# microsoft/VidTok

Hardware: NVIDIA H100
Metric: frames/sec encode+decode, kl_causal_488 17x256x256 (higher is better)
Workload: dtype bf16

## Files before the change

### vidtok_b200/csrc/conv_tc.cu

```cuda
#include <cuda.h>

#include <cstdio>
#include <cstdlib>
#include <cstring>
#include <mutex>
#include <string>
#include <type_traits>

#include "common.cuh"
#include "kernels.h"
#include "tc_host.h"
#include "tc_ptx.cuh"

namespace vt {

namespace {

thread_local std::string g_tc_err;

struct TcParams {
  int B, To, Ho, Wo, Co, Ti;
  int BW, BH, BT;
  int tilesW, tilesH, tilesT;
  int num_n_tiles, BN;
// ... 7 lines not shown
  int res_mode;
  const bf16* res;
  long long rsB, rsT, rsH, rsW;
  int resT, res_t_mode, res_pool_off;
  const bf16* res_cache;
  float ra, rb;
  void* out;
  long long osB, osT, osH, osW, osC;
  int out_f32;
  int Co_real;
  int w_batched;
  int ln_mode, ln_silu;
  const float* ln_gamma;
  const float* ln_beta;
  void* out2;
  int res_mma;
  int halo, hP, a_stages;
  uint32_t halo_bytes;
  int split, a_lo, b_lo, o_lo;
  float acc_scale;
  int kparts;
  int reg_mode, reg_zc, reg_sample;
  const float* reg_noise;
  float* reg_z;
  int* reg_idx;
  double* reg_kl;
  FsqConst reg_fsq;
  uint32_t misc_off;
  int stage_out;
  uint32_t stage_smem;
  uint32_t stage_off;
  int half_dim, half_ext;
  int relu;
};

struct TcMaps {
  CUtensorMap a[4];
  CUtensorMap c;
  CUtensorMap b;
  CUtensorMap r;
  CUtensorMap e;
  CUtensorMap o, o2;
};

constexpr int kConsumerWarps = 8;
constexpr int kProducerWarp = kConsumerWarps;
constexpr int kThreads = (kConsumerWarps + 4) * 32;
constexpr int kABytes = 128 * 128;
constexpr uint32_t kBarTurn = 3, kBarBias = 5, kBarStage = 7;
constexpr uint32_t kStageOutBytes = 64 * 128;

__host__ __device__ constexpr bool ping_pong(int BN, bool split) { return !split && (BN == 64 || BN == 128); }

using namespace tcx;

struct TileCoord {
  int b, t0, h0, w0, n0;
};
__device__ __forceinline__ TileCoord decode_tile(const TcParams& p, long long tile) {
  TileCoord c;
  const int nt = (int)(tile % p.num_n_tiles);
  long long m = tile / p.num_n_tiles;
  const int tw = (int)(m % p.tilesW); m /= p.tilesW;
  const int th = (int)(m % p.tilesH); m /= p.tilesH;
  const int tt = (int)(m % p.tilesT);
  c.b = (int)(m / p.tilesT);
  c.t0 = tt * p.BT; c.h0 = th * p.BH; c.w0 = tw * p.BW; c.n0 = nt * p.BN;
  return c;
}
__device__ __forceinline__ bool tap_time(const TcParams& p, const TileCoord& tc, int a, int& tv, bool& from_cache) {
  tv = (tc.t0 + p.to_off) * p.st + a - p.pt;
  from_cache = false;
  if (tv + p.BT <= 0) {
    if (p.t_mode == 0) return false;
    if (p.t_mode == 1) { tv = 0; return true; }
    from_cache = true;
    tv = p.cacheT + tv;
    return true;
  }
  return true;
}
__device__ __forceinline__ int tile_taps(const TcParams& p, const TileCoord& tc) {
  int n = 0;
  for (int a = 0; a < p.kt; ++a) {
    int tv;
    bool from_cache;
    if (tap_time(p, tc, a, tv, from_cache)) ++n;
  }
  return n;
}

__device__ __forceinline__ float quad_sum(float v) {
  v += __shfl_xor_sync(0xffffffffu, v, 1);
  v += __shfl_xor_sync(0xffffffffu, v, 2);
  return v;
}

template <int BN, bool kSplit, bool kStage = false>
__global__ void __launch_bounds__(kThreads, 1)
conv_tc_kernel(const __grid_constant__ TcMaps maps, const TcParams p) {
  extern __shared__ uint8_t smem_raw[];
  const uint32_t smem_base = (smem_u32(smem_raw) + 1023u) & ~1023u;
  uint8_t* smem_gen = smem_raw + (smem_base - smem_u32(smem_raw));
  const int warp = threadIdx.x >> 5, lane = threadIdx.x & 31;
  const uint32_t a_bytes = kABytes;
  constexpr uint32_t b_bytes = (uint32_t)BN * 128u;
  constexpr uint32_t kPl = kSplit ? 2u : 1u;
  const uint32_t stage_bytes = kPl * (p.halo ? b_bytes : a_bytes + b_bytes);
  const uint32_t win_bytes = kPl * p.halo_bytes;
  const uint32_t ring_base = smem_base + (p.halo ? (uint32_t)p.a_stages * win_bytes : 0u);
  const uint32_t bar_base = ring_base + p.stages * stage_bytes + p.stage_smem;
  auto full_bar = [&](int s) { return bar_base + 8u * s; };
  auto empty_bar = [&](int s) { return bar_base + 8u * (p.stages + s); };
// ... 171 lines not shown
    pend_stage = stage;
    pend_win = last_of_window;
    if (++stage == nstages) { stage = 0; phase ^= 1u; }
  };

  const int rbase = (kPingPong ? 0 : 64 * g) + 16 * wq + (lane >> 2);
  const int cq = 2 * (lane & 3);
  const bool res_direct = (p.res_mode == 1 && !p.res_mma);
  const bool store_a = (p.ln_mode != 1);
  const float inv_n = 1.0f / (float)BN;
  int last_n0 = -1;
  uint32_t cbuf = 1;

  int owner = 0;
  for (long long tile = blockIdx.x; tile < p.num_tiles; tile += gridDim.x, owner ^= 1) {
    const TileCoord tc = decode_tile(p, tile);
    if constexpr (kPingPong) {
      if (owner != g) {
        const int taps = tile_taps(p, tc);
        stage += taps * nsp * num_kc + res_steps;
        if ((stage / nstages) & 1) phase ^= 1u;
        stage %= nstages;
        if (halo) {
          const int nw = taps * num_kc + res_steps;
          sA += nw;
          if ((sA / p.a_stages) & 1) phA ^= 1u;
          sA %= p.a_stages;
          sR = (sR + nw) % p.a_stages;
        }
        continue;
      }
      if (tile != blockIdx.x) named_bar_sync(kBarTurn + g, kConsumerWarps * 32);
    }
    uint32_t G = 0xFFFFFFFFu;
    if constexpr (kSum) {
      if (p.kparts > 1) {
        const uint32_t nk = (uint32_t)(tile_taps(p, tc) * nsp * num_kc + res_steps);
        G = (nk + (uint32_t)p.kparts - 1u) / (uint32_t)p.kparts;
      }
#pragma unroll
      for (int i = 0; i < R; ++i) sum[i] = 0.f;
    }
    uint32_t ks = 0, accum = 0;
    auto step = [&](bool a_from_stage, uint32_t a_addr, bool res, bool last_of_window) {
      if constexpr (kSum) {
        if (ks > 0 && ks % G == 0) {
          wgmma_wait<0>();
          acc_fence(acc[0]);
          release();
#pragma unroll
          for (int i = 0; i < R; ++i) sum[i] += acc[0][i];
          accum = 0;
        }
      }
      kstep(a_from_stage, a_addr, accum, res, last_of_window);
      accum = 1;
      ++ks;
    };
    for (int a = 0; a < p.kt; ++a) {
      int tv;
      bool from_cache;
      if (!tap_time(p, tc, a, tv, from_cache)) continue;
      if (halo) {
        for (int kc = 0; kc < num_kc; ++kc) {
          mbar_wait(fullA_bar(sA), phA);
          const uint32_t win = smem_base + (uint32_t)sA * win_bytes + a_row_off;
// ... 19 lines not shown
      if (tile + gridDim.x < p.num_tiles) named_bar_arrive(kBarTurn + (g ^ 1), kConsumerWarps * 32);
    }
    wgmma_wait<0>();
#pragma unroll
    for (int hf = 0; hf < kHalves; ++hf) acc_fence(acc[hf]);
    release();
    if constexpr (kSum) {
#pragma unroll
      for (int i = 0; i < R; ++i) acc[0][i] += sum[i];
    }

    if (tc.n0 != last_n0) {
      last_n0 = tc.n0;
      cbuf ^= 1u;
      constexpr int nthr = kPingPong ? 128 : kConsumerWarps * 32;
      float* b_ = sbias + ((kPingPong ? 2 * g : 0) + cbuf) * 768;
      for (int i = threadIdx.x % nthr; i < BN; i += nthr) {
        b_[i] = (p.bias && tc.n0 + i < p.Co_real) ? p.bias[tc.n0 + i] : 0.f;
        if (p.ln_mode) { const float sc = (p.ln_silu && !kSplit) ? 0.5f : 1.0f; b_[256 + i] = sc * p.ln_gamma[tc.n0 + i]; b_[512 + i] = sc * p.ln_beta[tc.n0 + i]; }
      }
      named_bar_sync(kPingPong ? kBarBias + g : 1u, nthr);
    }
    const float* bias_s = sbias + ((kPingPong ? 2 * g : 0) + cbuf) * 768;
    const float* gamma_s = bias_s + 256;
    const float* beta_s = bias_s + 512;

#pragma unroll
    for (int hf = 0; hf < kHalves; ++hf) {
      float (&acc_h)[R] = acc[hf];
      int row0 = rbase + 64 * hf;
      asm volatile("" : "+r"(row0));
      bool valid[2];
      long long ooff[2];
      auto row_geom = [&](int row, int& t, int& h, int& w) {
        const int dw = halo ? (row & 7) : row % p.BW;
        const int dh = halo ? (row >> 3) : (row / p.BW) % p.BH;
        const int dt = halo ? 0 : row / (p.BW * p.BH);
        t = tc.t0 + dt; h = tc.h0 + dh; w = tc.w0 + dw;
        return (t < p.To) && (h < p.Ho) && (w < p.Wo);
      };
#pragma unroll
      for (int r = 0; r < 2; ++r) {
        int t, h, w;
        valid[r] = row_geom(row0 + 8 * r, t, h, w);
        ooff[r] = (long long)tc.b * p.osB + (long long)t * p.osT + (long long)h * p.osH + (long long)w * p.osW;
      }
      auto res_pair = [&](const bf16* rp, int c, float& x0, float& x1) {
        const uint32_t hw = *reinterpret_cast<const uint32_t*>(rp + c);
        if constexpr (kSplit) {
          const uint32_t lw = *reinterpret_cast<const uint32_t*>(rp + p.o_lo + c);
          x0 = f16_lo(hw) + f16_lo(lw);
          x1 = f16_hi(hw) + f16_hi(lw);
        } else {
          x0 = bf16_lo(hw);
          x1 = bf16_hi(hw);
        }
      };
#pragma unroll
      for (int j = 0; j < BN / 8; ++j) {
        const int c = 8 * j + cq;
#pragma unroll
        for (int e = 0; e < 4; ++e) {
          float f = kSplit ? fmaf(acc_h[4 * j + e], p.acc_scale, bias_s[c + (e & 1)]) : acc_h[4 * j + e] + bias_s[c + (e & 1)];
          if (p.rb != 1.0f) f *= p.rb;
          acc_h[4 * j + e] = f;
        }
      }
      if (res_direct || p.res_mode == 3) {
#pragma unroll
        for (int r = 0; r < 2; ++r) {
          int t, h, w;
          if (!row_geom(row0 + 8 * r, t, h, w)) continue;
          const bf16* r0 = nullptr;
          const bf16* r1 = nullptr;
          const bf16* r2 = nullptr;
          if (res_direct) {
            r0 = p.res + (long long)tc.b * p.rsB + (long long)t * p.rsT + (long long)h * p.rsH + (long long)w * p.rsW + tc.n0;
          } else {
            const long long sp = (long long)tc.b * p.rsB + (long long)h * p.rsH + (long long)w * p.rsW + tc.n0;
            const int ta = 2 * t - 1 + p.res_pool_off, tb = ta + 1, tcn = ta + 2;
            if (ta >= 0) r0 = p.res + sp + (long long)ta * p.rsT;
            else if (p.res_t_mode == 1) r0 = p.res + sp;
            else if (p.res_t_mode == 2) r0 = p.res_cache + (((long long)tc.b * p.Ho + h) * p.Wo + w) * (long long)p.Co * (kSplit ? 2 : 1) + tc.n0;
            if (tb < p.resT) r1 = p.res + sp + (long long)tb * p.rsT;
            if (tcn < p.resT) r2 = p.res + sp + (long long)tcn * p.rsT;
          }
#pragma unroll
          for (int j = 0; j < BN / 8; ++j) {
            const int c = 8 * j + cq;
            if (res_direct) {
              float x0, x1;
              res_pair(r0, c, x0, x1);
              acc_h[4 * j + 2 * r] = fmaf(p.ra, x0, acc_h[4 * j + 2 * r]);
              acc_h[4 * j + 2 * r + 1] = fmaf(p.ra, x1, acc_h[4 * j + 2 * r + 1]);
            } else {
              float s0 = 0.f, s1 = 0.f, x0, x1;
              if (r0) { res_pair(r0, c, x0, x1); s0 += x0; s1 += x1; }
              if (r1) { res_pair(r1, c, x0, x1); s0 += x0; s1 += x1; }
              if (r2) { res_pair(r2, c, x0, x1); s0 += x0; s1 += x1; }
              const float s3 = p.ra * (1.0f / 3.0f);
              acc_h[4 * j + 2 * r] = fmaf(s3, s0, acc_h[4 * j + 2 * r]);
              acc_h[4 * j + 2 * r + 1] = fmaf(s3, s1, acc_h[4 * j + 2 * r + 1]);
            }
          }
        }
// ... 119 lines not shown
              reserve();
#pragma unroll
              for (int r = 0; r < 2; ++r)
#pragma unroll
                for (int u = 0; u < 8; ++u) put_s(r, u, pack_bf16x2(acc_h[4 * (8 * k + u) + 2 * r], acc_h[4 * (8 * k + u) + 2 * r + 1]));
              send(&maps.o, k);
            }
          }
          if (p.ln_mode) {
            const CUtensorMap* nmap = p.ln_mode == 1 ? &maps.o : &maps.o2;
#pragma unroll
            for (int k = 0; k < BN / 64; ++k) {
              reserve();
#pragma unroll
              for (int r = 0; r < 2; ++r)
#pragma unroll
                for (int u = 0; u < 8; ++u) {
                  const int j = 8 * k + u, c = 8 * j + cq;
                  float y0 = fmaf(fmaf(acc_h[4 * j + 2 * r], rstd[r], nmr[r]), gamma_s[c], beta_s[c]);
                  float y1 = fmaf(fmaf(acc_h[4 * j + 2 * r + 1], rstd[r], nmr[r]), gamma_s[c + 1], beta_s[c + 1]);
                  if (p.ln_silu) {
                    y0 = fmaf(y0, tanh_approx(y0), y0);
                    y1 = fmaf(y1, tanh_approx(y1), y1);
                  }
                  put_s(r, u, pack_bf16x2(y0, y1));
                }
              send(nmap, k);
            }
          }
          continue;
        }
      }

      auto put = [&](void* optr, int r, int c, float y0, float y1) {
        bf16* o = reinterpret_cast<bf16*>(optr) + ooff[r] + tc.n0 + c;
        if constexpr (kSplit) {
          const uint32_t hw = pack_f16x2(y0, y1);
          *reinterpret_cast<uint32_t*>(o) = hw;
          *reinterpret_cast<uint32_t*>(o + p.o_lo) = pack_f16x2(y0 - f16_lo(hw), y1 - f16_hi(hw));
        } else {
          *reinterpret_cast<uint32_t*>(o) = pack_bf16x2(y0, y1);
        }
      };
      if constexpr (kSplit) {
        if (store_a) {
#pragma unroll
          for (int r = 0; r < 2; ++r)
            if (valid[r])
#pragma unroll
              for (int j = 0; j < BN / 8; ++j) put(p.out, r, 8 * j + cq, acc_h[4 * j + 2 * r], acc_h[4 * j + 2 * r + 1]);
        }
        if (p.ln_mode) {
          void* nout = p.ln_mode == 1 ? p.out : p.out2;
#pragma unroll
          for (int r = 0; r < 2; ++r) {
            float s = 0.f;
#pragma unroll
            for (int j = 0; j < BN / 8; ++j) s += acc_h[4 * j + 2 * r] + acc_h[4 * j + 2 * r + 1];
            const float mean = quad_sum(s) * inv_n;
            float q = 0.f;
#pragma unroll
            for (int j = 0; j < BN / 8; ++j) {
              const float d0 = acc_h[4 * j + 2 * r] - mean, d1 = acc_h[4 * j + 2 * r + 1] - mean;
              q = fmaf(d0, d0, q);
              q = fmaf(d1, d1, q);
            }
            const float rstd = 1.0f / sqrtf(quad_sum(q) * inv_n + 1e-6f);
            if (!valid[r]) continue;
#pragma unroll
            for (int j = 0; j < BN / 8; ++j) {
              const int c = 8 * j + cq;
              float y0 = (acc_h[4 * j + 2 * r] - mean) * rstd * gamma_s[c] + beta_s[c];
              float y1 = (acc_h[4 * j + 2 * r + 1] - mean) * rstd * gamma_s[c + 1] + beta_s[c + 1];
              if (p.ln_silu) { y0 = silu_tc(y0); y1 = silu_tc(y1); }
              put(nout, r, c, y0, y1);
            }
          }
        }
      } else {
#pragma unroll
        for (int r = 0; r < 2; ++r) {
          float s = 0.f, q = 0.f;
#pragma unroll
          for (int j = 0; j < BN / 8; ++j) {
            const float f0 = acc_h[4 * j + 2 * r], f1 = acc_h[4 * j + 2 * r + 1];
            s += f0 + f1;
            q = fmaf(f0, f0, q);
            q = fmaf(f1, f1, q);
            const uint32_t kp = pack_bf16x2(f0, f1);
            if (store_a && valid[r]) *reinterpret_cast<uint32_t*>(reinterpret_cast<bf16*>(p.out) + ooff[r] + tc.n0 + 8 * j + cq) = kp;
            acc_h[4 * j + 2 * r] = bf16_lo(kp);
            acc_h[4 * j + 2 * r + 1] = bf16_hi(kp);
          }
          if (!p.ln_mode) continue;
          const float mean = quad_sum(s) * inv_n;
          float var = fmaf(-mean, mean, quad_sum(q) * inv_n);
          var = var < 0.f ? 0.f : var;
          const float rstd = rsqrtf(var + 1e-6f);
          const float nmr = -mean * rstd;
          if (!valid[r]) continue;
          void* nout = p.ln_mode == 1 ? p.out : p.out2;
#pragma unroll
          for (int j = 0; j < BN / 8; ++j) {
            const int c = 8 * j + cq;
            float y0 = fmaf(fmaf(acc_h[4 * j + 2 * r], rstd, nmr), gamma_s[c], beta_s[c]);
            float y1 = fmaf(fmaf(acc_h[4 * j + 2 * r + 1], rstd, nmr), gamma_s[c + 1], beta_s[c + 1]);
            if (p.ln_silu) {
              y0 = fmaf(y0, tanh_approx(y0), y0);
              y1 = fmaf(y1, tanh_approx(y1), y1);
            }
            put(nout, r, c, y0, y1);
          }
        }
      }
    }
  }
  if (kStage && (threadIdx.x & 127) == 0) bulk_wait<0>();
}

__global__ void fill_identity_kernel(bf16* e, int f16, float value) {
  const int r = blockIdx.x, c = threadIdx.x;
  if (f16) reinterpret_cast<__half*>(e)[r * 256 + c] = __float2half_rn(r == c ? value : 0.0f);
  else e[r * 256 + c] = __float2bfloat16_rn(r == c ? value : 0.0f);
}

bool choose_tile(const ConvP& p, int rows, int& BW, int& BH, int& BT) {
  const bool allow_bt = (p.st == 1) && (p.t_mode == 0);
  long long best = -1;
  auto ceil_to = [](int v, int b) { return (long long)((v + b - 1) / b) * b; };
  for (int bw = 128; bw >= 8; bw >>= 1) {
    for (int bh = rows / bw; bh >= 1; bh >>= 1) {
      if (bh > 256) continue;
      const int bt = rows / (bw * bh);
      if (bt > 1 && !allow_bt) continue;
      if (bt > 16) continue;
      const long long padded = ceil_to(p.Wo, bw) * ceil_to(p.Ho, bh) * ceil_to(p.To, bt);
      const long long cost = padded * 1024 + (long long)(bw > 16 ? bw - 16 : 16 - bw) * 4 + (bt - 1);
      if (best < 0 || cost < best) { best = cost; BW = bw; BH = bh; BT = bt; }
    }
  }
  return best >= 0;
}
int choose_bn(int Co) {
  for (int bn = 256; bn >= 32; bn >>= 1)
// ... 84 lines not shown
  if (rc == 1) rc = plan(false, bn_pref);
  if (rc == 1 && !need_row) rc = plan(false, 128);
  if (rc == 1) return no("not enough shared memory for 2 stages");
  if (rc != 0) return false;
  bool ident_ok = true;
  if (split) {
    const float ws = p.acc_scale != 0.f ? 1.0f / p.acc_scale : 1.0f;
    t.ident_s = ilogbf(ws);
    ident_ok = t.ident_s >= 0 && t.ident_s <= 15 && ldexpf(1.0f, t.ident_s) == ws;
  }
  t.res_mma = (ident_ok && p.res_mode == 1 && p.ra == 1.0f && p.rb == 1.0f && t.BN % 64 == 0 && p.Co % 64 == 0 && p.rsW % 8 == 0 &&
               p.rsH % 8 == 0 && p.rsT % 8 == 0 && p.rsB % 8 == 0 && (((uintptr_t)p.res) & 15) == 0) ? 1 : 0;
  *out = t;
  return true;
}

cudaError_t launch_conv_tc(const TcPlan& pl, const bf16* x, const bf16* w_nk, void* out, cudaStream_t s, long long w_batch_stride) {
  if (!tmap_encoder()) { g_tc_err = "cuTensorMapEncodeTiled unavailable"; return cudaErrorNotSupported; }
  const ConvP& p = pl.p;
  const TcRegFusion& reg = pl.reg;
  const bool split = p.split != 0;
  const int cw = split ? 2 : 1;
  if (reg.mode ? (!reg.z || (reg.mode == 1 && (!reg.kl_acc || (reg.sample && !reg.noise)))) : !out) { g_tc_err = "null output"; return cudaErrorInvalidValue; }
  if (p.t_mode == 2 && (!p.cache || p.cacheT <= 0)) { g_tc_err = "cache mode without cache"; return cudaErrorInvalidValue; }
  int dev = 0;
  const cudaError_t dev_err = current_device(dev);
  if (dev_err != cudaSuccess) { g_tc_err = "no current device, or its index is out of range"; return dev_err; }
  const int Co_pad = (p.Co + 31) / 32 * 32, Kpad = p.kt * p.kh * p.kw * p.Ci;
  TcParams t;
  memset(&t, 0, sizeof(t));
  t.BW = pl.BW; t.BH = pl.BH; t.BT = pl.BT; t.BN = pl.BN;
  t.halo = pl.halo; t.hP = pl.hP; t.a_stages = pl.a_stages; t.halo_bytes = pl.halo_bytes;
  t.stages = pl.stages; t.misc_off = pl.misc_off; t.kparts = pl.kparts; t.res_mma = pl.res_mma;
  t.stage_smem = pl.stage_out ? 2 * kStageOutBytes : 0;
  t.stage_off = (uint32_t)pl.a_stages * pl.halo_bytes + (uint32_t)pl.stages * (uint32_t)((pl.halo ? 0 : kABytes) + pl.BN * 128);
  t.stage_out = (pl.stage_out && ((uintptr_t)out & 15) == 0 && ((uintptr_t)pl.ln.out2 & 15) == 0) ? 1 : 0;
  t.tilesW = (p.Wo + t.BW - 1) / t.BW; t.tilesH = (p.Ho + t.BH - 1) / t.BH; t.tilesT = (p.To + t.BT - 1) / t.BT;
  t.num_n_tiles = Co_pad / t.BN;
  t.num_tiles = (long long)p.B * t.tilesT * t.tilesH * t.tilesW * t.num_n_tiles;
  t.split = split ? 1 : 0; t.a_lo = p.Ci; t.b_lo = Kpad; t.o_lo = pl.o_lo ? pl.o_lo : p.Co;
  t.acc_scale = (split && p.acc_scale != 0.f) ? p.acc_scale : 1.0f;
  t.B = p.B; t.To = p.To; t.Ho = p.Ho; t.Wo = p.Wo; t.Co = p.Co; t.Ti = p.Ti;
  t.kt = p.kt; t.kh = p.kh; t.kw = p.kw; t.Ci = p.Ci; t.num_kc = p.Ci / 64;
  t.st = p.st; t.pt = p.pt; t.ph = p.ph; t.pw = p.pw; t.to_off = p.to_off; t.sp = p.sh;
  t.t_mode = p.t_mode; t.cacheT = p.cacheT;
  t.bias = p.bias; t.res_mode = p.res_mode; t.res = (const bf16*)p.res;
  t.rsB = p.rsB; t.rsT = p.rsT; t.rsH = p.rsH; t.rsW = p.rsW; t.resT = p.resT; t.res_t_mode = p.res_t_mode; t.res_pool_off = p.res_pool_off;
  t.res_cache = (const bf16*)p.res_cache; t.ra = p.ra; t.rb = p.rb;
  t.out = out; t.osB = p.osB; t.osT = p.osT; t.osH = p.osH; t.osW = p.osW; t.osC = p.osC;
  t.out_f32 = (pl.tout == DT_F32) ? 1 : 0;
  t.Co_real = p.Co;
  t.ln_mode = pl.ln.mode; t.ln_silu = pl.ln.silu ? 1 : 0; t.ln_gamma = pl.ln.gamma; t.ln_beta = pl.ln.beta; t.out2 = pl.ln.out2;
  if (reg.mode) {
    t.reg_mode = reg.mode; t.reg_zc = reg.zc; t.reg_sample = reg.sample; t.reg_noise = reg.noise; t.reg_z = reg.z;
    t.reg_idx = reg.indices; t.reg_kl = reg.kl_acc;
    if (reg.mode == 2) t.reg_fsq = make_fsq_const(reg.zc, reg.fsq_levels);
  }
  t.w_batched = pl.w_batches > 1 ? 1 : 0;
  t.relu = p.relu ? 1 : 0;

  TcMaps maps;
  auto encode_act = [&](CUtensorMap* m, const bf16* base, int Wn, int Hn, long long sw_, long long sh_, int Tn, long long st_, long long bs) -> bool {
    cuuint64_t dims[5] = {(cuuint64_t)(cw * p.Ci), (cuuint64_t)Wn, (cuuint64_t)Hn, (cuuint64_t)Tn, (cuuint64_t)p.B};
    cuuint64_t strides[4] = {(cuuint64_t)sw_ * 2, (cuuint64_t)sh_ * 2, (cuuint64_t)st_ * 2, (cuuint64_t)bs * 2};
    cuuint32_t box[5] = {64, (cuuint32_t)t.BW, (cuuint32_t)t.BH, (cuuint32_t)t.BT, 1};
    if (t.halo) { box[1] = (cuuint32_t)t.hP; box[2] = (cuuint32_t)(16 + p.kh - 1); }
    return encode_tmap_16b(m, 5, base, dims, strides, box, "activation", g_tc_err);
  };
  if (p.sh == 1) {
    if (!encode_act(&maps.a[0], x, p.Wi, p.Hi, p.isW, p.isH, p.Ti, p.isT, p.isB)) return cudaErrorInvalidValue;
    maps.a[1] = maps.a[2] = maps.a[3] = maps.a[0];
  } else {
    for (int hp = 0; hp < 2; ++hp)
      for (int wp = 0; wp < 2; ++wp)
        if (!encode_act(&maps.a[hp * 2 + wp], x + (long long)hp * p.isH + (long long)wp * p.isW, (p.Wi - wp + 1) / 2,
                        (p.Hi - hp + 1) / 2, 2 * p.isW, 2 * p.isH, p.Ti, p.isT, p.isB))
          return cudaErrorInvalidValue;
  }
  if (p.t_mode == 2) {
    if (!encode_act(&maps.c, (const bf16*)p.cache, p.Wi, p.Hi, p.isW, p.isH, p.cacheT, p.isT, (long long)p.cacheT * p.Hi * p.Wi * p.Ci * cw)) return cudaErrorInvalidValue;
  } else {
// ... 81 lines not shown
```

### vidtok_b200/csrc/tblock_tc.cu

```cuda
#include <cuda.h>

#include <cstdio>
#include <cstring>
#include <string>

#include "common.cuh"
#include "kernels.h"
#include "tc_host.h"
#include "tc_ptx.cuh"

namespace vt {

namespace {
using namespace tcx;

thread_local std::string g_tb_err;
constexpr int kC = 128;
constexpr int kKc = kC / 64;
constexpr uint32_t kTile = 128 * 128;
constexpr int kHSlots = 3;
constexpr int kConsumerWarps = 8;
constexpr int kProducerWarp = kConsumerWarps;
constexpr int kThreadsTb = (kConsumerWarps + 4) * 32;

struct TbParams {
  int B, T, H, W;
  int BW, BH;
  int tilesW, tilesH;
  long long num_strips;
  int stages;
  const float* bias1;
  const float* bias2;
  const float* g2;
  const float* b2;
  int ln_out, ln_out_silu;
  const float* g3;
  const float* b3;
  const bf16* x;
  bf16* out;
  bf16* out2;
  const bf16* n1;
  int cached_in;
  const bf16* cn1_in;
  const bf16* ch_in;
  bf16* cn1_out;
  bf16* ch_out;
};
struct TbMaps {
  CUtensorMap n1, w1, w2, cn1;
  CUtensorMap x, out;
};

__device__ __forceinline__ float quad_sum(float v) {
  v += __shfl_xor_sync(0xffffffffu, v, 1);
  v += __shfl_xor_sync(0xffffffffu, v, 2);
  return v;
}

template <bool kCache>
__global__ void __launch_bounds__(kThreadsTb, 1) tblock_tc_kernel(const __grid_constant__ TbMaps maps, const TbParams p) {
  extern __shared__ uint8_t smem_raw[];
  const uint32_t smem_base = (smem_u32(smem_raw) + 1023u) & ~1023u;
  uint8_t* smem_gen = smem_raw + (smem_base - smem_u32(smem_raw));
  const int warp = threadIdx.x >> 5, lane = threadIdx.x & 31;
  const uint32_t h_base = smem_base;
  const uint32_t ring_base = h_base + kHSlots * kKc * kTile;
  const uint32_t stage_bytes = 2u * kTile;
  const uint32_t bar_base = ring_base + (uint32_t)p.stages * stage_bytes;
  auto full_bar = [&](int s) { return bar_base + 8u * s; };
  auto empty_bar = [&](int s) { return bar_base + 8u * (p.stages + s); };
  auto x_bar = [&](int g) { return bar_base + 16u * p.stages + 8u * g; };
  float* cst = reinterpret_cast<float*>(smem_gen + (bar_base - smem_base) + 16u * p.stages + 16u);

// ... 200 lines not shown
      finish();
      mbar_wait(x_bar(g), xphase);
      xphase ^= 1u;
      const uint32_t xslot = slot_of(t - 2);
#pragma unroll
      for (int r = 0; r < 2; ++r) {
        const long long off = (pos0[r] + (long long)t * frame) * kC;
        const int row = rbase + 8 * r;
        uint8_t* xs = smem_gen + (xslot - smem_base);
        float s = 0.f, q = 0.f;
#pragma unroll
        for (int j = 0; j < kC / 8; ++j) {
          const int c = 8 * j + cq;
          const int cc = c & 63;
          uint32_t* xo = reinterpret_cast<uint32_t*>(xs + (c >> 6) * kTile + swz128_unit(row, cc >> 3) + (cc & 7) * 2);
          const uint32_t xw = *xo;
          const float f0 = acc[4 * j + 2 * r] + bias2[c] + bf16_lo(xw), f1 = acc[4 * j + 2 * r + 1] + bias2[c + 1] + bf16_hi(xw);
          s += f0 + f1;
          q = fmaf(f0, f0, q);
          q = fmaf(f1, f1, q);
          const uint32_t kp = pack_bf16x2(f0, f1);
          *xo = kp;
          acc[4 * j + 2 * r] = bf16_lo(kp);
          acc[4 * j + 2 * r + 1] = bf16_hi(kp);
        }
        if (!p.ln_out) continue;
        const float mean = quad_sum(s) * (1.0f / kC);
        float var = fmaf(-mean, mean, quad_sum(q) * (1.0f / kC));
        var = var < 0.f ? 0.f : var;
        const float rstd = rsqrtf(var + 1e-6f);
        const float nmr = -mean * rstd;
        bf16* o2 = p.out2 + off;
#pragma unroll
        for (int j = 0; j < kC / 8; ++j) {
          const int c = 8 * j + cq;
          float y0 = fmaf(fmaf(acc[4 * j + 2 * r], rstd, nmr), g3[c], b3[c]);
          float y1 = fmaf(fmaf(acc[4 * j + 2 * r + 1], rstd, nmr), g3[c + 1], b3[c + 1]);
          if (p.ln_out_silu) {
            y0 = fmaf(y0, tanh_approx(y0), y0);
            y1 = fmaf(y1, tanh_approx(y1), y1);
          }
          *reinterpret_cast<uint32_t*>(o2 + c) = pack_bf16x2(y0, y1);
        }
      }
      fence_async_smem();
      wg_sync();
      if (gtid == 0) {
        for (int kc = 0; kc < kKc; ++kc)
          tma_store_5d(&maps.out, xslot + (uint32_t)g * 64u * 128u + (uint32_t)kc * kTile, kc * 64, box_w, box_h, t, b);
        bulk_commit();
      }
    }
    if (kCache) {
      for (int j = 0; j < 2; ++j) {
        const int tv = p.T - 2 + j;
        for (int i = gtid; i < 64 * 16; i += 128) {
          int row;
          const long long off = cache_pos(i, j, row);
          const long long pix = off - (((long long)b * 2 + j) * frame) * kC;
          uint4 hv = make_uint4(0u, 0u, 0u, 0u), nv = hv;
          if (tv >= 0 || front) hv = *ring_unit(slot_of(tv), row, (i & 15) * 8);
          if (tv >= 0) nv = *reinterpret_cast<const uint4*>(p.n1 + (((long long)b * p.T + tv) * frame) * kC + pix);
          else if (front) nv = *reinterpret_cast<const uint4*>(p.cn1_in + (((long long)b * 2 + tv + 2) * frame) * kC + pix);
          *reinterpret_cast<uint4*>(p.ch_out + off) = hv;
          *reinterpret_cast<uint4*>(p.cn1_out + off) = nv;
        }
      }
    }
  }
  if (gtid == 0) bulk_wait<0>();
}

bool strip_box(int H, int W, int& BW, int& BH) {
  for (int bw = 128; bw >= 1; bw >>= 1) {
    if (W % bw != 0) continue;
// ... 2 lines not shown
  }
  return false;
}
}

const char* tblock_tc_last_error() { return g_tb_err.c_str(); }

bool tblock_tc_supported(int B, int T, int H, int W, int C) {
  g_tb_err.clear();
  if (C != kC) { g_tb_err = "C != 128"; return false; }
  if (B <= 0 || T <= 0) { g_tb_err = "empty"; return false; }
  int BW, BH;
  if (!strip_box(H, W, BW, BH)) { g_tb_err = "H x W not tileable by a 128-position box"; return false; }
  return true;
}

cudaError_t launch_tblock_tc(const bf16* n1, const bf16* x, const bf16* w1, const float* bias1, const float* gamma2,
                             const float* beta2, const bf16* w2, const float* bias2, bf16* out, bf16* out2,
                             const float* gamma_out, const float* beta_out, bool out_silu, int B, int T, int H, int W,
                             cudaStream_t s, const TbCache* cache) {
  g_tb_err.clear();
  if (!tmap_encoder()) { g_tb_err = "cuTensorMapEncodeTiled unavailable"; return cudaErrorNotSupported; }
  TbParams p;
  memset(&p, 0, sizeof(p));
  if (!strip_box(H, W, p.BW, p.BH)) { g_tb_err = "H x W not tileable"; return cudaErrorInvalidValue; }
  p.B = B; p.T = T; p.H = H; p.W = W;
  p.tilesW = W / p.BW; p.tilesH = H / p.BH;
  p.num_strips = (long long)B * p.tilesH * p.tilesW;
  p.bias1 = bias1; p.bias2 = bias2; p.g2 = gamma2; p.b2 = beta2;
  p.ln_out = (out2 && gamma_out && beta_out) ? 1 : 0;
  p.ln_out_silu = out_silu ? 1 : 0;
  p.g3 = gamma_out; p.b3 = beta_out;
  p.x = x; p.out = out; p.out2 = out2;
  if (cache) {
    if (!cache->n1_out || !cache->h_out || (!cache->n1_in != !cache->h_in)) { g_tb_err = "cache: both outputs, and both or no inputs"; return cudaErrorInvalidValue; }
    p.n1 = n1;
    p.cached_in = cache->n1_in ? 1 : 0;
    p.cn1_in = cache->n1_in; p.ch_in = cache->h_in; p.cn1_out = cache->n1_out; p.ch_out = cache->h_out;
  }
  const size_t fixed = 1024 + (size_t)kHSlots * kKc * kTile + 16 + 6 * kC * 4;
  const size_t budget = 225 * 1024;
  int stages = (int)((budget - fixed) / (2 * kTile + 16));
  if (stages > 4) stages = 4;
  p.stages = stages;
  const size_t smem = fixed + (size_t)stages * (2 * kTile + 16);
  TbMaps maps;
  {
    cuuint64_t dims[5] = {(cuuint64_t)kC, (cuuint64_t)W, (cuuint64_t)H, (cuuint64_t)T, (cuuint64_t)B};
    cuuint64_t strides[4] = {(cuuint64_t)kC * 2, (cuuint64_t)W * kC * 2, (cuuint64_t)H * W * kC * 2, (cuuint64_t)T * H * W * kC * 2};
    cuuint32_t box[5] = {64, (cuuint32_t)p.BW, (cuuint32_t)p.BH, 1, 1};
    if (!encode_tmap_16b(&maps.n1, 5, n1, dims, strides, box, "n1", g_tb_err)) return cudaErrorInvalidValue;
    maps.cn1 = maps.n1;
    const int bw = p.BW < 64 ? p.BW : 64;
    cuuint32_t box64[5] = {64, (cuuint32_t)bw, (cuuint32_t)(64 / bw), 1, 1};
    for (int i = 0; i < 2; ++i)
      if (!encode_tmap_16b(i ? &maps.out : &maps.x, 5, i ? (const void*)out : x, dims, strides, box64, "x / out", g_tb_err))
        return cudaErrorInvalidValue;
    if (p.cached_in) {
      dims[3] = 2;
      strides[3] = 2ull * H * W * kC * 2;
      if (!encode_tmap_16b(&maps.cn1, 5, p.cn1_in, dims, strides, box, "n1 cache", g_tb_err)) return cudaErrorInvalidValue;
    }
  }
  for (int i = 0; i < 2; ++i) {
    cuuint64_t dims[3] = {(cuuint64_t)(3 * kC), (cuuint64_t)kC, 1};
    cuuint64_t strides[2] = {(cuuint64_t)(3 * kC) * 2, (cuuint64_t)(3 * kC) * kC * 2};
// ... 26 lines not shown
```

### vidtok_b200/csrc/tc_ptx.cuh

```cuda
#pragma once
#include <cuda.h>
#include <cuda_bf16.h>
#include <cuda_fp16.h>
#include <stdint.h>

namespace vt {
namespace tcx {
__device__ __forceinline__ uint32_t smem_u32(const void* p) { return (uint32_t)__cvta_generic_to_shared(p); }

__device__ __forceinline__ void mbar_init(uint32_t bar, uint32_t count) {
  asm volatile("mbarrier.init.shared::cta.b64 [%0], %1;" ::"r"(bar), "r"(count) : "memory");
}
__device__ __forceinline__ void mbar_expect_tx(uint32_t bar, uint32_t bytes) {
  asm volatile("mbarrier.arrive.expect_tx.shared::cta.b64 _, [%0], %1;" ::"r"(bar), "r"(bytes) : "memory");
}
__device__ __forceinline__ void mbar_arrive(uint32_t bar) {
  asm volatile("mbarrier.arrive.shared::cta.b64 _, [%0];" ::"r"(bar) : "memory");
}
__device__ __forceinline__ bool mbar_try_wait(uint32_t bar, uint32_t parity) {
  uint32_t ok;
  asm volatile(
      "{\n\t"
      ".reg .pred p;\n\t"
      "mbarrier.try_wait.parity.shared::cta.b64 p, [%1], %2;\n\t"
// ... 11 lines not shown
    if (clock64() - t0 > 8000000000LL) __trap();
  }
}
__device__ __forceinline__ void tma_load_5d(uint32_t dst, const CUtensorMap* map, uint32_t bar, int c0, int c1, int c2,
                                            int c3, int c4) {
  asm volatile(
      "cp.async.bulk.tensor.5d.shared::cluster.global.mbarrier::complete_tx::bytes [%0], [%1, {%3, %4, %5, %6, %7}], [%2];"
      ::"r"(dst), "l"(map), "r"(bar), "r"(c0), "r"(c1), "r"(c2), "r"(c3), "r"(c4)
      : "memory");
}
__device__ __forceinline__ void tma_load_3d(uint32_t dst, const CUtensorMap* map, uint32_t bar, int c0, int c1, int c2) {
  asm volatile(
      "cp.async.bulk.tensor.3d.shared::cluster.global.mbarrier::complete_tx::bytes [%0], [%1, {%3, %4, %5}], [%2];"
      ::"r"(dst), "l"(map), "r"(bar), "r"(c0), "r"(c1), "r"(c2)
      : "memory");
}
__device__ __forceinline__ void tma_store_5d(const CUtensorMap* map, uint32_t src, int c0, int c1, int c2, int c3, int c4) {
  asm volatile("cp.async.bulk.tensor.5d.global.shared::cta.bulk_group [%0, {%2, %3, %4, %5, %6}], [%1];"
               ::"l"(map), "r"(src), "r"(c0), "r"(c1), "r"(c2), "r"(c3), "r"(c4)
               : "memory");
}
__device__ __forceinline__ void bulk_commit() { asm volatile("cp.async.bulk.commit_group;" ::: "memory"); }
template <int kPending>
__device__ __forceinline__ void bulk_wait_read() { asm volatile("cp.async.bulk.wait_group.read %0;" ::"n"(kPending) : "memory"); }
template <int kPending>
__device__ __forceinline__ void bulk_wait() { asm volatile("cp.async.bulk.wait_group %0;" ::"n"(kPending) : "memory"); }
__device__ __forceinline__ void fence_async_smem() { asm volatile("fence.proxy.async.shared::cta;" ::: "memory"); }
__device__ __forceinline__ void named_bar_sync(uint32_t id, uint32_t threads) {
  asm volatile("bar.sync %0, %1;" ::"r"(id), "r"(threads) : "memory");
}
__device__ __forceinline__ void named_bar_arrive(uint32_t id, uint32_t threads) {
  asm volatile("bar.arrive %0, %1;" ::"r"(id), "r"(threads) : "memory");
}
__device__ __forceinline__ void prefetch_tmap(const CUtensorMap* map) {
  asm volatile("prefetch.tensormap [%0];" ::"l"(map) : "memory");
}
__device__ __forceinline__ bool elect_one() {
  uint32_t pred;
  asm volatile(
      "{\n\t"
      ".reg .pred P1;\n\t"
      "elect.sync _|P1, 0xffffffff;\n\t"
      "selp.u32 %0, 1, 0, P1;\n\t"
      "}"
      : "=r"(pred));
  return pred != 0;
}

__device__ __forceinline__ void wgmma_fence() { asm volatile("wgmma.fence.sync.aligned;" ::: "memory"); }
__device__ __forceinline__ void wgmma_commit() { asm volatile("wgmma.commit_group.sync.aligned;" ::: "memory"); }
template <int kPending>
__device__ __forceinline__ void wgmma_wait() { asm volatile("wgmma.wait_group.sync.aligned %0;" ::"n"(kPending) : "memory"); }
template <int R>
__device__ __forceinline__ void acc_fence(float (&d)[R]) {
#pragma unroll
  for (int i = 0; i < R; ++i) asm volatile("" : "+f"(d[i])::"memory");
}

__device__ __forceinline__ uint32_t desc_lo(uint32_t saddr) { return ((saddr & 0x3FFFFu) >> 4) | (1u << 16); }
__device__ __forceinline__ uint32_t desc_hi(uint32_t sbo) { return (sbo >> 4) | (1u << 30); }
__device__ __forceinline__ uint64_t desc(uint32_t lo, uint32_t hi) { return ((uint64_t)hi << 32) | lo; }
__device__ __forceinline__ uint32_t swz128_unit(int row, int u) { return (uint32_t)row * 128u + (uint32_t)((u ^ (row & 7)) << 4); }

__device__ __forceinline__ void wgmma_32_bf16(float (&d)[16], uint64_t da, uint64_t db, uint32_t scale_d) {
  asm volatile(
      "{\n\t.reg .pred p;\n\t"
// ... 170 lines not shown
#pragma unroll
  for (int i = 0; i < 4; ++i) {
    f[2 * i] = __low2float(h[i]);
    f[2 * i + 1] = __high2float(h[i]);
  }
}
__device__ __forceinline__ uint32_t pack_bf16x2(float lo, float hi) {
  uint32_t r;
  asm("cvt.rn.bf16x2.f32 %0, %1, %2;" : "=r"(r) : "f"(hi), "f"(lo));
  return r;
}
__device__ __forceinline__ float tanh_approx(float x) { float t; asm("tanh.approx.f32 %0, %1;" : "=f"(t) : "f"(x)); return t; }
__device__ __forceinline__ uint32_t pack_f16x2(float lo, float hi) {
  lo = fminf(fmaxf(lo, -65504.0f), 65504.0f);
  hi = fminf(fmaxf(hi, -65504.0f), 65504.0f);
  uint32_t r;
  asm("cvt.rn.f16x2.f32 %0, %1, %2;" : "=r"(r) : "f"(hi), "f"(lo));
  return r;
}
__device__ __forceinline__ float f16_lo(uint32_t w) { return __half2float(__ushort_as_half((unsigned short)(w & 0xFFFFu))); }
__device__ __forceinline__ float f16_hi(uint32_t w) { return __half2float(__ushort_as_half((unsigned short)(w >> 16))); }
__device__ __forceinline__ void unpack8h(const uint4& u, float (&f)[8]) {
  const __half2* h = reinterpret_cast<const __half2*>(&u);
#pragma unroll
  for (int i = 0; i < 4; ++i) {
    const float2 v = __half22float2(h[i]);
    f[2 * i] = v.x;
    f[2 * i + 1] = v.y;
  }
}
__device__ __forceinline__ float bf16_lo(uint32_t w) { float f; asm("mov.b32 %0, %1;" : "=f"(f) : "r"(w << 16)); return f; }
__device__ __forceinline__ float bf16_hi(uint32_t w) { float f; asm("mov.b32 %0, %1;" : "=f"(f) : "r"(w & 0xFFFF0000u)); return f; }

}
}
```

Measured before the change: 468.4.

## Vectorize epilogue residual loads and output stores via quad transposes; prefetch residuals

Epilogue stores and direct residual loads now use 16-byte accesses. Each quad of threads first exchanges its packed bf16 words with warp shuffles so every thread holds eight contiguous channels, replacing many 4-byte scattered accesses. Residual rows are also prefetched into L2 before the main MMA loop. The cost is extra shuffle instructions and register pressure, and the vector paths are guarded by host-side 16-byte alignment checks.

```diff
diff --git a/vidtok_b200/csrc/conv_tc.cu b/vidtok_b200/csrc/conv_tc.cu
--- a/vidtok_b200/csrc/conv_tc.cu
+++ b/vidtok_b200/csrc/conv_tc.cu
@@ -63,6 +63,7 @@
   uint32_t stage_off;
   int half_dim, half_ext;
   int relu;
+  int vec_out, vec_res;
 };
 
 struct TcMaps {
@@ -110,6 +111,14 @@
     return true;
   }
   return true;
+}
+__device__ __forceinline__ bool tile_row(const TcParams& p, const TileCoord& tc, int row, int& t, int& h, int& w) {
+  const bool halo = p.halo != 0;
+  const int dw = halo ? (row & 7) : row % p.BW;
+  const int dh = halo ? (row >> 3) : (row / p.BW) % p.BH;
+  const int dt = halo ? 0 : row / (p.BW * p.BH);
+  t = tc.t0 + dt; h = tc.h0 + dh; w = tc.w0 + dw;
+  return (t < p.To) && (h < p.Ho) && (w < p.Wo);
 }
 __device__ __forceinline__ int tile_taps(const TcParams& p, const TileCoord& tc) {
   int n = 0;
@@ -347,6 +356,21 @@
       }
       if (tile != blockIdx.x) named_bar_sync(kBarTurn + g, kConsumerWarps * 32);
     }
+    if (res_direct) {
+#pragma unroll
+      for (int hf = 0; hf < kHalves; ++hf)
+#pragma unroll
+        for (int r = 0; r < 2; ++r) {
+          int row = rbase + 64 * hf + 8 * r, t, h, w;
+          asm volatile("" : "+r"(row));
+          if (!tile_row(p, tc, row, t, h, w)) continue;
+          const bf16* rp = p.res + (long long)tc.b * p.rsB + (long long)t * p.rsT + (long long)h * p.rsH + (long long)w * p.rsW + tc.n0;
+          for (int l = lane & 3; l < (BN + 63) / 64; l += 4) {
+            prefetch_l2(rp + 64 * l);
+            if constexpr (kSplit) prefetch_l2(rp + p.o_lo + 64 * l);
+          }
+        }
+    }
     uint32_t G = 0xFFFFFFFFu;
     if constexpr (kSum) {
       if (p.kparts > 1) {
@@ -432,13 +456,7 @@
       asm volatile("" : "+r"(row0));
       bool valid[2];
       long long ooff[2];
-      auto row_geom = [&](int row, int& t, int& h, int& w) {
-        const int dw = halo ? (row & 7) : row % p.BW;
-        const int dh = halo ? (row >> 3) : (row / p.BW) % p.BH;
-        const int dt = halo ? 0 : row / (p.BW * p.BH);
-        t = tc.t0 + dt; h = tc.h0 + dh; w = tc.w0 + dw;
-        return (t < p.To) && (h < p.Ho) && (w < p.Wo);
-      };
+      auto row_geom = [&](int row, int& t, int& h, int& w) { return tile_row(p, tc, row, t, h, w); };
 #pragma unroll
       for (int r = 0; r < 2; ++r) {
         int t, h, w;
@@ -466,11 +484,42 @@
           acc_h[4 * j + e] = f;
         }
       }
+      constexpr bool kVecRes = !kStage && !(kSplit && BN == 256);
+      const bool vec_res = kVecRes && p.vec_res && res_direct;
       if (res_direct || p.res_mode == 3) {
 #pragma unroll
         for (int r = 0; r < 2; ++r) {
           int t, h, w;
-          if (!row_geom(row0 + 8 * r, t, h, w)) continue;
+          const bool ok = row_geom(row0 + 8 * r, t, h, w);
+          if (vec_res) {
+            const bf16* rp = p.res + (long long)tc.b * p.rsB + (long long)t * p.rsT + (long long)h * p.rsH + (long long)w * p.rsW + tc.n0 + 4 * cq;
+#pragma unroll
+            for (int k = 0; k < BN / 32; ++k) {
+              uint32_t hw[4] = {0u, 0u, 0u, 0u}, lw[4] = {0u, 0u, 0u, 0u};
+              if (ok) {
+                const uint4 u = *reinterpret_cast<const uint4*>(rp + 32 * k);
+                hw[0] = u.x; hw[1] = u.y; hw[2] = u.z; hw[3] = u.w;
+                if constexpr (kSplit) {
+                  const uint4 v = *reinterpret_cast<const uint4*>(rp + p.o_lo + 32 * k);
+                  lw[0] = v.x; lw[1] = v.y; lw[2] = v.z; lw[3] = v.w;
+                }
+              }
+              quad_transpose(hw);
+              if constexpr (kSplit) quad_transpose(lw);
+              if (ok) {
+#pragma unroll
+                for (int i = 0; i < 4; ++i) {
+                  const int j = 4 * k + i;
+                  const float x0 = kSplit ? f16_lo(hw[i]) + f16_lo(lw[i]) : bf16_lo(hw[i]);
+                  const float x1 = kSplit ? f16_hi(hw[i]) + f16_hi(lw[i]) : bf16_hi(hw[i]);
+                  acc_h[4 * j + 2 * r] = fmaf(p.ra, x0, acc_h[4 * j + 2 * r]);
+                  acc_h[4 * j + 2 * r + 1] = fmaf(p.ra, x1, acc_h[4 * j + 2 * r + 1]);
+                }
+              }
+            }
+            continue;
+          }
+          if (!ok) continue;
           const bf16* r0 = nullptr;
           const bf16* r1 = nullptr;
           const bf16* r2 = nullptr;
@@ -656,17 +705,13 @@
         }
       }
 
-      auto put = [&](void* optr, int r, int c, float y0, float y1) {
-        bf16* o = reinterpret_cast<bf16*>(optr) + ooff[r] + tc.n0 + c;
-        if constexpr (kSplit) {
+      if constexpr (kSplit) {
+        auto put = [&](void* optr, int r, int c, float y0, float y1) {
+          bf16* o = reinterpret_cast<bf16*>(optr) + ooff[r] + tc.n0 + c;
           const uint32_t hw = pack_f16x2(y0, y1);
           *reinterpret_cast<uint32_t*>(o) = hw;
           *reinterpret_cast<uint32_t*>(o + p.o_lo) = pack_f16x2(y0 - f16_lo(hw), y1 - f16_hi(hw));
-        } else {
-          *reinterpret_cast<uint32_t*>(o) = pack_bf16x2(y0, y1);
-        }
-      };
-      if constexpr (kSplit) {
+        };
         if (store_a) {
 #pragma unroll
           for (int r = 0; r < 2; ++r)
@@ -702,19 +747,34 @@
           }
         }
       } else {
+        auto put_words = [&](void* optr, int r, int k, uint32_t (&wv)[4]) {
+          bf16* o = reinterpret_cast<bf16*>(optr) + ooff[r] + tc.n0;
+          if (p.vec_out) {
+            quad_transpose(wv);
+            if (valid[r]) st_global_v4(o + 32 * k + 4 * cq, wv);
+          } else if (valid[r]) {
+#pragma unroll
+            for (int i = 0; i < 4; ++i) *reinterpret_cast<uint32_t*>(o + 8 * (4 * k + i) + cq) = wv[i];
+          }
+        };
 #pragma unroll
         for (int r = 0; r < 2; ++r) {
           float s = 0.f, q = 0.f;
 #pragma unroll
-          for (int j = 0; j < BN / 8; ++j) {
-            const float f0 = acc_h[4 * j + 2 * r], f1 = acc_h[4 * j + 2 * r + 1];
-            s += f0 + f1;
-            q = fmaf(f0, f0, q);
-            q = fmaf(f1, f1, q);
-            const uint32_t kp = pack_bf16x2(f0, f1);
-            if (store_a && valid[r]) *reinterpret_cast<uint32_t*>(reinterpret_cast<bf16*>(p.out) + ooff[r] + tc.n0 + 8 * j + cq) = kp;
-            acc_h[4 * j + 2 * r] = bf16_lo(kp);
-            acc_h[4 * j + 2 * r + 1] = bf16_hi(kp);
+          for (int k = 0; k < BN / 32; ++k) {
+            uint32_t wv[4];
+#pragma unroll
+            for (int i = 0; i < 4; ++i) {
+              const int j = 4 * k + i;
+              const float f0 = acc_h[4 * j + 2 * r], f1 = acc_h[4 * j + 2 * r + 1];
+              s += f0 + f1;
+              q = fmaf(f0, f0, q);
+              q = fmaf(f1, f1, q);
+              wv[i] = pack_bf16x2(f0, f1);
+              acc_h[4 * j + 2 * r] = bf16_lo(wv[i]);
+              acc_h[4 * j + 2 * r + 1] = bf16_hi(wv[i]);
+            }
+            if (store_a) put_words(p.out, r, k, wv);
           }
           if (!p.ln_mode) continue;
           const float mean = quad_sum(s) * inv_n;
@@ -722,18 +782,22 @@
           var = var < 0.f ? 0.f : var;
           const float rstd = rsqrtf(var + 1e-6f);
           const float nmr = -mean * rstd;
-          if (!valid[r]) continue;
           void* nout = p.ln_mode == 1 ? p.out : p.out2;
 #pragma unroll
-          for (int j = 0; j < BN / 8; ++j) {
-            const int c = 8 * j + cq;
-            float y0 = fmaf(fmaf(acc_h[4 * j + 2 * r], rstd, nmr), gamma_s[c], beta_s[c]);
-            float y1 = fmaf(fmaf(acc_h[4 * j + 2 * r + 1], rstd, nmr), gamma_s[c + 1], beta_s[c + 1]);
-            if (p.ln_silu) {
-              y0 = fmaf(y0, tanh_approx(y0), y0);
-              y1 = fmaf(y1, tanh_approx(y1), y1);
-            }
-            put(nout, r, c, y0, y1);
+          for (int k = 0; k < BN / 32; ++k) {
+            uint32_t wv[4];
+#pragma unroll
+            for (int i = 0; i < 4; ++i) {
+              const int j = 4 * k + i, c = 8 * j + cq;
+              float y0 = fmaf(fmaf(acc_h[4 * j + 2 * r], rstd, nmr), gamma_s[c], beta_s[c]);
+              float y1 = fmaf(fmaf(acc_h[4 * j + 2 * r + 1], rstd, nmr), gamma_s[c + 1], beta_s[c + 1]);
+              if (p.ln_silu) {
+                y0 = fmaf(y0, tanh_approx(y0), y0);
+                y1 = fmaf(y1, tanh_approx(y1), y1);
+              }
+              wv[i] = pack_bf16x2(y0, y1);
+            }
+            put_words(nout, r, k, wv);
           }
         }
       }
@@ -884,9 +948,12 @@
   t.BW = pl.BW; t.BH = pl.BH; t.BT = pl.BT; t.BN = pl.BN;
   t.halo = pl.halo; t.hP = pl.hP; t.a_stages = pl.a_stages; t.halo_bytes = pl.halo_bytes;
   t.stages = pl.stages; t.misc_off = pl.misc_off; t.kparts = pl.kparts; t.res_mma = pl.res_mma;
+  auto aligned16 = [](const void* q) { return ((uintptr_t)q & 15) == 0; };
+  const bool out16 = aligned16(out) && aligned16(pl.ln.out2);
   t.stage_smem = pl.stage_out ? 2 * kStageOutBytes : 0;
   t.stage_off = (uint32_t)pl.a_stages * pl.halo_bytes + (uint32_t)pl.stages * (uint32_t)((pl.halo ? 0 : kABytes) + pl.BN * 128);
-  t.stage_out = (pl.stage_out && ((uintptr_t)out & 15) == 0 && ((uintptr_t)pl.ln.out2 & 15) == 0) ? 1 : 0;
+  t.stage_out = (pl.stage_out && out16) ? 1 : 0;
+  t.vec_out = out16 ? 1 : 0;
   t.tilesW = (p.Wo + t.BW - 1) / t.BW; t.tilesH = (p.Ho + t.BH - 1) / t.BH; t.tilesT = (p.To + t.BT - 1) / t.BT;
   t.num_n_tiles = Co_pad / t.BN;
   t.num_tiles = (long long)p.B * t.tilesT * t.tilesH * t.tilesW * t.num_n_tiles;
@@ -899,6 +966,7 @@
   t.bias = p.bias; t.res_mode = p.res_mode; t.res = (const bf16*)p.res;
   t.rsB = p.rsB; t.rsT = p.rsT; t.rsH = p.rsH; t.rsW = p.rsW; t.resT = p.resT; t.res_t_mode = p.res_t_mode; t.res_pool_off = p.res_pool_off;
   t.res_cache = (const bf16*)p.res_cache; t.ra = p.ra; t.rb = p.rb;
+  t.vec_res = (aligned16(p.res) && (p.rsB | p.rsT | p.rsH | p.rsW) % 8 == 0 && (!split || t.o_lo % 8 == 0)) ? 1 : 0;
   t.out = out; t.osB = p.osB; t.osT = p.osT; t.osH = p.osH; t.osW = p.osW; t.osC = p.osC;
   t.out_f32 = (pl.tout == DT_F32) ? 1 : 0;
   t.Co_real = p.Co;
diff --git a/vidtok_b200/csrc/tblock_tc.cu b/vidtok_b200/csrc/tblock_tc.cu
--- a/vidtok_b200/csrc/tblock_tc.cu
+++ b/vidtok_b200/csrc/tblock_tc.cu
@@ -39,6 +39,7 @@
   const bf16* x;
   bf16* out;
   bf16* out2;
+  int vec_out2;
   const bf16* n1;
   int cached_in;
   const bf16* cn1_in;
@@ -305,15 +306,26 @@
         const float nmr = -mean * rstd;
         bf16* o2 = p.out2 + off;
 #pragma unroll
-        for (int j = 0; j < kC / 8; ++j) {
-          const int c = 8 * j + cq;
-          float y0 = fmaf(fmaf(acc[4 * j + 2 * r], rstd, nmr), g3[c], b3[c]);
-          float y1 = fmaf(fmaf(acc[4 * j + 2 * r + 1], rstd, nmr), g3[c + 1], b3[c + 1]);
-          if (p.ln_out_silu) {
-            y0 = fmaf(y0, tanh_approx(y0), y0);
-            y1 = fmaf(y1, tanh_approx(y1), y1);
+        for (int k = 0; k < kC / 32; ++k) {
+          uint32_t wv[4];
+#pragma unroll
+          for (int i = 0; i < 4; ++i) {
+            const int j = 4 * k + i, c = 8 * j + cq;
+            float y0 = fmaf(fmaf(acc[4 * j + 2 * r], rstd, nmr), g3[c], b3[c]);
+            float y1 = fmaf(fmaf(acc[4 * j + 2 * r + 1], rstd, nmr), g3[c + 1], b3[c + 1]);
+            if (p.ln_out_silu) {
+              y0 = fmaf(y0, tanh_approx(y0), y0);
+              y1 = fmaf(y1, tanh_approx(y1), y1);
+            }
+            wv[i] = pack_bf16x2(y0, y1);
           }
-          *reinterpret_cast<uint32_t*>(o2 + c) = pack_bf16x2(y0, y1);
+          if (p.vec_out2) {
+            quad_transpose(wv);
+            st_global_v4(o2 + 32 * k + 4 * cq, wv);
+          } else {
+#pragma unroll
+            for (int i = 0; i < 4; ++i) *reinterpret_cast<uint32_t*>(o2 + 8 * (4 * k + i) + cq) = wv[i];
+          }
         }
       }
       fence_async_smem();
@@ -382,6 +394,7 @@
   p.ln_out_silu = out_silu ? 1 : 0;
   p.g3 = gamma_out; p.b3 = beta_out;
   p.x = x; p.out = out; p.out2 = out2;
+  p.vec_out2 = ((uintptr_t)out2 & 15) == 0 ? 1 : 0;
   if (cache) {
     if (!cache->n1_out || !cache->h_out || (!cache->n1_in != !cache->h_in)) { g_tb_err = "cache: both outputs, and both or no inputs"; return cudaErrorInvalidValue; }
     p.n1 = n1;
diff --git a/vidtok_b200/csrc/tc_ptx.cuh b/vidtok_b200/csrc/tc_ptx.cuh
--- a/vidtok_b200/csrc/tc_ptx.cuh
+++ b/vidtok_b200/csrc/tc_ptx.cuh
@@ -67,6 +67,7 @@
 __device__ __forceinline__ void named_bar_arrive(uint32_t id, uint32_t threads) {
   asm volatile("bar.arrive %0, %1;" ::"r"(id), "r"(threads) : "memory");
 }
+__device__ __forceinline__ void prefetch_l2(const void* ptr) { asm volatile("prefetch.global.L2 [%0];" ::"l"(ptr)); }
 __device__ __forceinline__ void prefetch_tmap(const CUtensorMap* map) {
   asm volatile("prefetch.tensormap [%0];" ::"l"(map) : "memory");
 }
@@ -303,5 +304,22 @@
 __device__ __forceinline__ float bf16_lo(uint32_t w) { float f; asm("mov.b32 %0, %1;" : "=f"(f) : "r"(w << 16)); return f; }
 __device__ __forceinline__ float bf16_hi(uint32_t w) { float f; asm("mov.b32 %0, %1;" : "=f"(f) : "r"(w & 0xFFFF0000u)); return f; }
 
-}
-}
+__device__ __forceinline__ void quad_transpose(uint32_t (&w)[4]) {
+#pragma unroll
+  for (int m = 2; m >= 1; m >>= 1) {
+    const bool up = (threadIdx.x & m) != 0;
+#pragma unroll
+    for (int a = 0; a < 4; ++a) {
+      if (a & m) continue;
+      const uint32_t got = __shfl_xor_sync(0xffffffffu, up ? w[a] : w[a | m], m);
+      if (up) w[a] = got;
+      else w[a | m] = got;
+    }
+  }
+}
+__device__ __forceinline__ void st_global_v4(void* ptr, const uint32_t (&w)[4]) {
+  asm volatile("st.global.v4.b32 [%0], {%1, %2, %3, %4};" ::"l"(ptr), "r"(w[0]), "r"(w[1]), "r"(w[2]), "r"(w[3]) : "memory");
+}
+
+}
+}
```

Result: no change. 472.7 (median of 6 runs) (+0.9%).
